# patngnw/NewsRecommendation

Hardware: AMD Instinct MI355X
Metric: train impressions/sec @ batch 512, NRMS (higher is better)
Workload: dtype bf16; 1 GPU; NRMS train step (fwd+bwd+Adam), MIND-small shapes: title_len=30, history=50, npratio=4, 300-d word table; per_gpu_batch=512, global_batch=512, vocab_rows=30000, freeze_embedding=False, compact_history=False, dense_batch=False, feed=resident, deterministic=False, optimizer=flat bucket + HIP fused Adam, parallelism=dp1

## Files before the change

### newsrecommendation_amd/csrc/nr_gemm.hip

```cpp
#include <stdlib.h>

#include "nr_gemm.h"

namespace {

constexpr int BM = 128, BN = 128, BK = 32, NTHR = 256;
constexpr int SC = BN + 4;

template <typename T> struct TileCfg {
  static constexpr int CH = 16 / (int)sizeof(T);
  static constexpr int SK = BK + CH;
  static constexpr int CPR = BK / CH;
  static constexpr int NCH = BM * CPR / NTHR;
  static constexpr int RPC = BM / CH;
  static constexpr size_t STAGE_BYTES = (size_t)2 * 2 * BM * SK * sizeof(T);
};
constexpr size_t EPI_BYTES = (size_t)64 * SC * sizeof(float);

template <typename T> constexpr size_t smem_bytes() {
  return TileCfg<T>::STAGE_BYTES > EPI_BYTES ? TileCfg<T>::STAGE_BYTES : EPI_BYTES;
}

union Chunk {
  uint4 u;
// ... 1919 lines not shown
          const int row = u / xc, ch = u - row * xc;
          *reinterpret_cast<uint4*>(a.dx + (r0 + row) * a.lddx + ch * 8) = make_uint4(0, 0, 0, 0);
        }
      if (near)
        for (int u = lane; u < L * qc; u += 64) {
          const int row = u / qc, ch = u - row * qc;
          *reinterpret_cast<uint4*>(a.dpre + (r0 + row) * a.ldp + ch * 8) = make_uint4(0, 0, 0, 0);
        }
    }
    nsteps = run;
  } else {
    for (int c = tid; c < nsteps; c += 512) sList[c] = b0 + c * G;
  }
  for (int c = tid; c < 256; c += 512) {
    sW2[c] = c < q ? a.w2[c] : 0.f;
    sRedW[c] = 0.f;
  }
  const int wcol0 = wid * TPW * 16;
  bf16x8 bfr[TPW][KS2];
#pragma unroll
  for (int t = 0; t < TPW; ++t) {
    const bf16_t* brow = a.w1t + (size_t)min(wcol0 + t * 16 + fr, N - 1) * a.ldw1t + 8 * g;
#pragma unroll
    for (int s2 = 0; s2 < KS2; ++s2) bfr[t][s2] = *reinterpret_cast<const bf16x8*>(brow + 32 * s2);
  }
  __builtin_amdgcn_s_waitcnt(0x0F70);
  __syncthreads();
  float* prow_out = a.partial + (size_t)blockIdx.x * (q + 1);
  if (nsteps == 0) {
    for (int c = tid; c <= q; c += 512) prow_out[c] = 0.f;
    return;
  }

  const uint32_t dump_lds = lds0 + Cfg::DUMP + wid * 1024;
  uint4* dump_g = g_nt_dump + wid * 64 + lane;
  auto issue_stage = [&](int kk) {
    const uint32_t slot = lds0 + (kk % NS) * STAGE;
    const bool real = kk < nsteps;
    const int sq = real ? sList[kk] : 0;
    const int row0 = sq * L;
#pragma unroll
    for (int u = 0; u < PW; ++u) {
      const int p = wid + NW * u;
      if (real && p < EPIECES) {
        const int i = p / KS2, s2 = p - i * KS2;
        const bf16_t* rp = a.e + (size_t)min(row0 + 16 * i + prow, M - 1) * a.lde + c8;
        dma16(rp + min(32 * s2, q - 8 - c8), slot + p * 1024);
      } else if (real && p < EPIECES + Cfg::GPIECES) {
        const int j = p - EPIECES;
        dma16(a.g + (size_t)sq * a.ldg + min(256 * j + 4 * lane, N - 4), slot + p * 1024);
      } else {
        dma16(a.e + c8, dump_lds);
      }
    }
  };
  const int ks0 = wid, ks1 = wid + NW;
  auto load_seq = [&](int kk, bf16x8 (&xf)[RT][2], float& al) {
    const int row0 = sList[kk < nsteps ? kk : 0] * L;
#pragma unroll
    for (int i = 0; i < RT; ++i) {
      const bf16_t* rp = a.x + (size_t)min(row0 + 16 * i + fr, M - 1) * a.ldx;
      xf[i][0] = *reinterpret_cast<const bf16x8*>(rp + min(32 * ks0 + 8 * g, N - 8));
      xf[i][1] = *reinterpret_cast<const bf16x8*>(rp + min(32 * ks1 + 8 * g, N - 8));
    }
    const int rowa = sList[(kk >= 1 && kk - 1 < nsteps) ? kk - 1 : 0] * L;
    al = a.alpha[min(rowa + (lane & 31), M - 1)];
  };
  auto g_frag = [&](const float* grow, int ks, bf16x8& hi, bf16x8& lo) {
    const int k0 = 32 * ks + 8 * g;
    const bool ok = ks < KS && k0 < N;
    const f32x4 v0 = *reinterpret_cast<const f32x4*>(grow + min(k0, N - 8));
    const f32x4 v1 = *reinterpret_cast<const f32x4*>(grow + min(k0, N - 8) + 4);
#pragma unroll
    for (int e2 = 0; e2 < 8; ++e2) {
      const float v = ok ? (e2 < 4 ? v0[e2] : v1[e2 - 4]) : 0.f;
      const bf16_t h = (bf16_t)v;
      hi[e2] = h;
      lo[e2] = (bf16_t)(v - (float)h);
    }
  };
  auto sum32 = [&](float v) {
    v += __builtin_bit_cast(float, __builtin_amdgcn_update_dpp(0, __builtin_bit_cast(int, v), 0x128, 0xf, 0xf, false));
    v += __builtin_bit_cast(float, __builtin_amdgcn_update_dpp(0, __builtin_bit_cast(int, v), 0x124, 0xf, 0xf, false));
    v += __builtin_bit_cast(float, __builtin_amdgcn_update_dpp(0, __builtin_bit_cast(int, v), 0x122, 0xf, 0xf, false));
    v += __builtin_bit_cast(float, __builtin_amdgcn_update_dpp(0, __builtin_bit_cast(int, v), 0x121, 0xf, 0xf, false));
    return v + __shfl_xor(v, 16, 64);
  };
  const int offA = fr * 64 + ((g ^ swzP(fr)) << 4);
  const uint32_t inv_qc = (uint32_t)((0x100000000ull + (uint32_t)qc - 1) / (uint32_t)qc);
  int brow[2], bcc[2];
#pragma unroll
  for (int j = 0; j < 2; ++j) {
    const uint32_t u = (uint32_t)(tid + 512 * j);
    uint32_t r = __umulhi(u, inv_qc);
    if (r * (uint32_t)qc > u) --r;
    brow[j] = (int)r;
    bcc[j] = (int)(u - r * (uint32_t)qc);
  }

  bf16x8 xf[RT][2];
  float al_nb, al_cur = 0.f;
  float* myacc = reinterpret_cast<float*>(smem + Cfg::ACCW) + tid * 8;
#pragma unroll
  for (int j = 0; j < 2; ++j) {
    *reinterpret_cast<f32x4*>(myacc + j * 4096) = (f32x4){0.f, 0.f, 0.f, 0.f};
    *reinterpret_cast<f32x4*>(myacc + j * 4096 + 4) = (f32x4){0.f, 0.f, 0.f, 0.f};
  }
  float accb = 0.f;

#pragma unroll 1
  for (int kk = 0; kk < 2; ++kk) issue_stage(kk);
  load_seq(0, xf, al_nb);

#pragma unroll 1
  for (int k = 0; k < nsteps + 2; ++k) {
    if (k >= 2) asm volatile("s_waitcnt vmcnt(%0)" ::"n"(Cfg::STEADY) : "memory");
    else wait_vmcnt_le(k == 0 ? PW + Cfg::LOADS : Cfg::OPS + Cfg::LOADS);
    __builtin_amdgcn_s_barrier();
    issue_stage(k + 2);
    auto phase_a = [&]()     {
      const bool real = k < nsteps;
      const float* grow = reinterpret_cast<const float*>(smem + (k % NS) * STAGE + EPIECES * 1024);
      f32x4 da[RT];
#pragma unroll
      for (int i = 0; i < RT; ++i) da[i] = (f32x4){0.f, 0.f, 0.f, 0.f};
      if (real) {
#pragma unroll
        for (int j = 0; j < 2; ++j) {
          bf16x8 hi, lo;
          g_frag(grow, j == 0 ? ks0 : ks1, hi, lo);
#pragma unroll
          for (int i = 0; i < RT; ++i) {
            da[i] = __builtin_amdgcn_mfma_f32_16x16x32_bf16(hi, xf[i][j], da[i], 0, 0, 0);
            da[i] = __builtin_amdgcn_mfma_f32_16x16x32_bf16(lo, xf[i][j], da[i], 0, 0, 0);
          }
        }
      }
      if (g == 0) {
#pragma unroll
        for (int i = 0; i < RT; ++i) sPartA[((k & 1) * NW + wid) * 32 + 16 * i + fr] = da[i][0];
      }
      al_cur = al_nb;
      load_seq(k + 1, xf, al_nb);
    };
    auto phase_b = [&]()     {
      const int kp = k - 1;
      const bool real = kp >= 0 && kp < nsteps;
      const int row0 = real ? sList[kp] * L : 0;
      const bool in = (lane & 31) < L;
      const float alv = in ? al_cur : 0.f;
      const float* part = sPartA + ((kp & 1) * NW) * 32 + (lane & 31);
      float dA = 0.f;
#pragma unroll
      for (int w = 0; w < NW; ++w) dA += part[w * 32];
      dA = in ? dA : 0.f;
      const float tsum = sum32(alv * dA);
      const float ds = alv * (dA - tsum);
      if (wid == 0 && lane < 32) sAlpha[(kp & 3) * 32 + lane] = alv;
      if (real) accb += sum32(ds);
      char* st = smem + ((kp + NS) % NS) * STAGE;
#pragma unroll
      for (int j = 0; j < 2; ++j) {
        const int row = brow[j], cc = bcc[j];
        const bool valid = real && row < L;
        const int rc = min(row, L - 1);
        const float dsr = __shfl(ds, rc, 64);
        const int eoff = ((rc >> 4) * KS2 + (cc >> 2)) * 1024 + (rc & 15) * 64 + (((cc & 3) ^ swzP(rc & 15)) << 4);
        const bf16x8 ev = *reinterpret_cast<const bf16x8*>(st + eoff);
        const f32x4 wa = *reinterpret_cast<const f32x4*>(sW2 + cc * 8), wb = *reinterpret_cast<const f32x4*>(sW2 + cc * 8 + 4);
        bf16x8 o;
        f32x4 a0 = *reinterpret_cast<const f32x4*>(myacc + j * 4096), a1 = *reinterpret_cast<const f32x4*>(myacc + j * 4096 + 4);
#pragma unroll
        for (int e2 = 0; e2 < 8; ++e2) {
          const float f = (float)ev[e2], wv = e2 < 4 ? wa[e2] : wb[e2 - 4];
          o[e2] = (bf16_t)(dsr * wv * (1.f - f * f));
          const float p = valid ? dsr * f : 0.f;
          if (e2 < 4) a0[e2] += p;
          else a1[e2 - 4] += p;
        }
        *reinterpret_cast<f32x4*>(myacc + j * 4096) = a0;
        *reinterpret_cast<f32x4*>(myacc + j * 4096 + 4) = a1;
        if (valid) *reinterpret_cast<bf16x8*>(st + eoff) = o;
        uint4* dst = valid ? reinterpret_cast<uint4*>(a.dpre + (size_t)(row0 + row) * a.ldp + cc * 8) : dump_g;
        *dst = __builtin_bit_cast(uint4, o);
      }
    };
    auto phase_c = [&]()     {
      const int kc = k - 2;
      const bool real = kc >= 0 && kc < nsteps;
      const int row0 = real ? sList[kc] * L : 0;
      const char* st = smem + ((kc + NS) % NS) * STAGE;
      const float* grow = reinterpret_cast<const float*>(st + EPIECES * 1024);
#pragma unroll
      for (int i = 0; i < RT; ++i) {
        f32x4 acc[TPW];
#pragma unroll
        for (int t = 0; t < TPW; ++t) acc[t] = (f32x4){0.f, 0.f, 0.f, 0.f};
        if (real && wcol0 < N) {
#pragma unroll
          for (int s2 = 0; s2 < KS2; ++s2) {
            const bf16x8 af = *reinterpret_cast<const bf16x8*>(st + (i * KS2 + s2) * 1024 + offA);
#pragma unroll
            for (int t = 0; t < TPW; ++t) acc[t] = __builtin_amdgcn_mfma_f32_16x16x32_bf16(bfr[t][s2], af, acc[t], 0, 0, 0);
          }
        }
        const int ml = 16 * i + fr;
        const bool rok = real && ml < L;
        const float al = sAlpha[((kc + 4) & 3) * 32 + ml];
        bf16_t* crow = a.dx + (size_t)(row0 + ml) * a.lddx;
#pragma unroll
        for (int t = 0; t < TPW; t += 2) {
          uint2 pk[2];
#pragma unroll
          for (int h = 0; h < 2; ++h) {
            const int lc = wcol0 + (t + h) * 16 + 4 * g;
            const f32x4 gq = *reinterpret_cast<const f32x4*>(grow + lc);
            const f32x4 v = acc[t + h];
            const bf16x4 o = {(bf16_t)(v[0] + al * gq[0]), (bf16_t)(v[1] + al * gq[1]), (bf16_t)(v[2] + al * gq[2]), (bf16_t)(v[3] + al * gq[3])};
            pk[h] = __builtin_bit_cast(uint2, o);
          }
          const auto s0 = __builtin_amdgcn_permlane16_swap(pk[0].x, pk[1].x, false, false);
          const auto s1 = __builtin_amdgcn_permlane16_swap(pk[0].y, pk[1].y, false, false);
          const int col = wcol0 + (t + (g & 1)) * 16 + (g >> 1) * 8;
          uint4* dst = (rok && col + 8 <= N) ? reinterpret_cast<uint4*>(crow + col) : dump_g;
          *dst = make_uint4(s0[0], s1[0], s0[1], s1[1]);
        }
      }
    };
    if (wid < NW / 2) {
      phase_a();
      phase_b();
      phase_c();
    } else {
      phase_c();
      phase_a();
      phase_b();
    }
  }
#pragma unroll
  for (int j = 0; j < 2; ++j)
#pragma unroll
    for (int e2 = 0; e2 < 8; ++e2) atomicAdd(sRedW + bcc[j] * 8 + e2, myacc[j * 4096 + e2]);
  __syncthreads();
  for (int c = tid; c < q; c += 512) prow_out[c] = sRedW[c];
  if (tid == 0) prow_out[q] = accb;
}

template <int EPI, int NT16, bool PK, int WM>
int launch_nt_dma_w(const RowSrc& A, const void* B, int ldb, int M, int N, int K, const EpiArgs& ep, hipStream_t stream) {
  constexpr int DBM = 64 * WM, NP = DBM / 16 + NT16, STAGE = NP * 1024, NS = dma_ring_stages(STAGE, WM);
  constexpr size_t ring = (size_t)NS * STAGE, epi = (size_t)32 * (NT16 * 16 + 4) * sizeof(float);
  constexpr size_t epk = PK ? (size_t)128 * (NT16 * 16 + 8) * sizeof(bf16_t) : 0;
  constexpr size_t gtile = EPI == EPI_POOLBWD && PK ? (size_t)((12 * NT16 * 16 * 4 + 1023) / 1024) * 1024 + 1024
                                                    : ((EPI == EPI_SCATTER || EPI == EPI_STORE) ? 2048 : 1024);
  constexpr size_t smem0 = ring > epi ? ring : epi, smem1 = smem0 > epk ? smem0 : epk, smem = smem1 + gtile;
  auto kern = gemm_nt_dma_kernel<EPI, NT16, PK, WM>;
  NR_CHECK_HIP(hipFuncSetAttribute(reinterpret_cast<const void*>(kern), hipFuncAttributeMaxDynamicSharedMemorySize, (int)smem));
  const int tilesM = (M + DBM - 1) / DBM, nchunks = (N + NT16 * 16 - 1) / (NT16 * 16);
  const int grid = ((tilesM + 7) / 8) * 8 * nchunks;
  hipLaunchKernelGGL(kern, dim3(grid), dim3(128 * WM), smem, stream, (const bf16_t*)A.base, A.ld, (const bf16_t*)B, ldb, M, N, K, ep, nchunks);
  NR_CHECK_LAUNCH();
  return NR_OK;
}

template <int EPI, int NT16, bool PK>
int launch_nt_dma_p(const RowSrc& A, const void* B, int ldb, int M, int N, int K, const EpiArgs& ep, hipStream_t stream) {
  constexpr bool fits2 = 3 * (8 + NT16) * 1024 <= 78 * 1024;
  if (fits2 && (N <= 2 * NT16 * 16 || K <= 224)) return launch_nt_dma_w<EPI, NT16, PK, 2>(A, B, ldb, M, N, K, ep, stream);
  return launch_nt_dma_w<EPI, NT16, PK, 4>(A, B, ldb, M, N, K, ep, stream);
}

template <int EPI, int NT16>
int launch_nt_dma_t(const RowSrc& A, const void* B, int ldb, int M, int N, int K, const EpiArgs& ep, hipStream_t stream) {
  if (EPI != EPI_SCATTER && ep.out_dtype == NR_BF16) return launch_nt_dma_p<EPI, NT16, true>(A, B, ldb, M, N, K, ep, stream);
  return launch_nt_dma_p<EPI, NT16, false>(A, B, ldb, M, N, K, ep, stream);
}

template <int NT16>
int launch_nt_dma_e(const RowSrc& A, const void* B, int ldb, int M, int N, int K, int epi, const EpiArgs& ep, hipStream_t s) {
  switch (epi) {
    case EPI_STORE: return launch_nt_dma_t<EPI_STORE, NT16>(A, B, ldb, M, N, K, ep, s);
    case EPI_STORE_TANH: return launch_nt_dma_t<EPI_STORE_TANH, NT16>(A, B, ldb, M, N, K, ep, s);
    case EPI_POOLBWD: return launch_nt_dma_t<EPI_POOLBWD, NT16>(A, B, ldb, M, N, K, ep, s);
    case EPI_SCATTER: return launch_nt_dma_t<EPI_SCATTER, NT16>(A, B, ldb, M, N, K, ep, s);
  }
  nr_set_error("gemm_nt_dma: bad epilogue %d", epi);
  return NR_ERR_ARG;
}

namespace tn3 {
using tn2::swz_a;
using tn2::tr_frag;
constexpr int TBM = 32, NS = 4;
template <int WK, int NI> struct Geo {
  static constexpr int TBN = 32 * NI, TBK = 80 * WK, NT = 128 * WK, NW = 2 * WK, CHA = TBN / 8, CH = TBK / 8, SCW = TBK + 4;
  static constexpr int PA = TBM * CHA / 64, PBP = TBM * CH / 64, NP = PA + PBP, STAGE = NP * 1024;
  static constexpr size_t RING = (size_t)NS * STAGE, EPI = (size_t)64 * SCW * sizeof(float);
  static constexpr size_t SMEM = RING > EPI ? RING : EPI;
};
template <int WK> __device__ __forceinline__ int swz_b(int row, int chunk) {
  return WK == 2 ? chunk ^ (2 * ((row >> 3) & 1)) : chunk ^ (4 * ((row >> 1) & 1) + 2 * ((row >> 3) & 1));
}

template <int WK, int NI>
__global__ __launch_bounds__(128 * WK) void gemm_tn3_kernel(const bf16_t* __restrict__ dC, int ldc, const bf16_t* __restrict__ X,
                                                            int ldx, float* __restrict__ dW, int ldw, float* __restrict__ db,
                                                            int M, int N, int K, int Nstore, int Kstore, int tilesK, int ntile,
                                                            int nsplit, int rps, const int32_t* __restrict__ slab_list,
                                                            const int32_t* __restrict__ slab_count, int xgap, float* __restrict__ scratch) {
  using G = Geo<WK, NI>;
  constexpr int TBN = G::TBN, TBK = G::TBK, NT = G::NT, NW = G::NW, CHA = G::CHA, CH = G::CH, SCW = G::SCW, PA = G::PA, NP = G::NP,
                STAGE = G::STAGE;
  constexpr int PB = NP / NW, PX = NP % NW;
  extern __shared__ __attribute__((aligned(16))) char smem[];
  const bool det = nr_fix_on();
  float* sC = reinterpret_cast<float*>(smem);
  const uint32_t lds0 = (uint32_t)(size_t)(__attribute__((address_space(3))) char*)smem;

  const int b = blockIdx.x, xcd = b & 7, local = b >> 3;
  const int split = (local / ntile) * 8 + xcd, tile = local % ntile;
  if (split >= nsplit) return;
  const int tn = tile / tilesK, tk = tile % tilesK;
  const int n0 = tn * TBN, k0 = tk * TBK;
  __shared__ int sSlab[1024];
  const bool slabs = slab_list != nullptr, counted = !slabs && slab_count != nullptr;
  int mbeg = split * rps, nk, kbeg = 0;
  if (slabs || counted) {
    const int total = counted ? (*slab_count + TBM - 1) / TBM : *slab_count, per = (total + nsplit - 1) / nsplit;
    kbeg = split * per;
    nk = min(per, total - kbeg);
    if (nk <= 0) return;
    if (slabs) {
      for (int i = threadIdx.x; i < nk; i += blockDim.x) sSlab[i] = slab_list[kbeg + i];
      __syncthreads();
    }
    mbeg = 0;
  } else {
    const int mend = min(M, mbeg + rps);
    if (mbeg >= mend) return;
    nk = (mend - mbeg) / TBM;
  }
  const int tid = threadIdx.x, lane = tid & 63;
  const int wid = __builtin_amdgcn_readfirstlane(tid >> 6), wm = wid / WK, wn = wid % WK;
  const bool extra = wid < PX;
  const int pfirst = wid * PB + min(wid, PX);
  const bool db_wave = (db != nullptr) && (tk == 0) && (wn == wm);

  const bf16_t* src[PB + 1];
  size_t adv[PB + 1];
  int xrow[PB + 1];
#pragma unroll
  for (int t = 0; t < PB + 1; ++t) {
    const int p = pfirst + t;
    xrow[t] = -1;
    if (p < PA) {
      const int P = 64 * p + lane, row = P / CHA, cpos = P - row * CHA;
      const int col = min(n0 + swz_a(row, cpos) * 8, N - 8);
      src[t] = dC + (size_t)(mbeg + row) * ldc + col;
      adv[t] = (size_t)TBM * ldc;
    } else {
      const int P = 64 * (p - PA) + lane, row = min(P / CH, TBM - 1), cpos = P - (P / CH) * CH;
      const int col = min(k0 + swz_b<WK>(row, cpos) * 8, K - 8);
      src[t] = X + (size_t)(mbeg + row) * ldx + col;
      adv[t] = (size_t)TBM * ldx;
      xrow[t] = mbeg + row;
    }
  }
  const uint32_t ginv = xgap > 0 ? (uint32_t)((0x100000000ull + (uint32_t)xgap - 1) / (uint32_t)xgap) : 0u;
  auto issue = [&](int stage, int kt) {
    const size_t sl = slabs ? (size_t)sSlab[kt] : (size_t)(kbeg + kt);
#pragma unroll
    for (int t = 0; t < PB + 1; ++t)
      if (t < PB || extra) {
        size_t off = sl * adv[t];
        if (xgap > 0 && xrow[t] >= 0) {
          const uint32_t m = (uint32_t)sl * TBM + (uint32_t)xrow[t];
          uint32_t q = __umulhi(m, ginv);
          if (q * (uint32_t)xgap > m) --q;
          off += (size_t)q * ldx;
        }
        dma16(src[t] + off, lds0 + stage * STAGE + (pfirst + t) * 1024);
      }
  };
  auto wait_stages = [&](int stages) {
    if (extra) {
      if (stages >= 2) asm volatile("s_waitcnt vmcnt(%0)" ::"n"(2 * (PB + 1)) : "memory");
      else if (stages == 1) asm volatile("s_waitcnt vmcnt(%0)" ::"n"(PB + 1) : "memory");
      else asm volatile("s_waitcnt vmcnt(0)" ::: "memory");
    } else {
      if (stages >= 2) asm volatile("s_waitcnt vmcnt(%0)" ::"n"(2 * PB) : "memory");
      else if (stages == 1) asm volatile("s_waitcnt vmcnt(%0)" ::"n"(PB) : "memory");
      else asm volatile("s_waitcnt vmcnt(0)" ::: "memory");
    }
  };

  f32x4 acc[NI][5];
#pragma unroll
  for (int i = 0; i < NI; ++i)
#pragma unroll
    for (int j = 0; j < 5; ++j) acc[i][j] = (f32x4){0.f, 0.f, 0.f, 0.f};
  f32x4 accdb = (f32x4){0.f, 0.f, 0.f, 0.f};
  const bf16_t one = (bf16_t)1.f, zero = (bf16_t)0.f;

  const int g = lane >> 4, q = (lane & 15) >> 2, pp = lane & 3;
  const int r0 = 8 * g + q, r1 = r0 + 4, off = 4 * (pp & 1);
  const int a0 = r0 * TBN + off, a1 = r1 * TBN + off, ca = wm * 2 * NI + (pp >> 1);
  int ob0[5], ob1[5];
#pragma unroll
  for (int j = 0; j < 5; ++j) {
    const int chunk = (wn * 80 + j * 16) / 8 + (pp >> 1);
    ob0[j] = TBM * TBN + r0 * TBK + swz_b<WK>(r0, chunk) * 8 + off;
    ob1[j] = TBM * TBN + r1 * TBK + swz_b<WK>(r1, chunk) * 8 + off;
  }

#pragma unroll
  for (int s = 0; s < NS - 1; ++s)
    if (s < nk) issue(s, s);
  for (int kt = 0; kt < nk; ++kt) {
    wait_stages(min(NS - 2, nk - 1 - kt));
    __builtin_amdgcn_s_barrier();
    if (kt + NS - 1 < nk) issue((kt + NS - 1) % NS, kt + NS - 1);
    const bf16_t* st = reinterpret_cast<const bf16_t*>(smem + (kt % NS) * STAGE);
    bf16x8 bf[5];
#pragma unroll
    for (int j = 0; j < 5; ++j) bf[j] = tr_frag(st + ob0[j], st + ob1[j]);
#pragma unroll
    for (int i = 0; i < NI; ++i) {
      const bf16x8 af = tr_frag(st + a0 + swz_a(r0, ca + 2 * i) * 8, st + a1 + swz_a(r1, ca + 2 * i) * 8);
#pragma unroll
      for (int j = 0; j < 5; ++j) acc[i][j] = __builtin_amdgcn_mfma_f32_16x16x32_bf16(af, bf[j], acc[i][j], 0, 0, 0);
      if (db_wave) {
        const bf16_t v = (lane & 15) == i ? one : zero;
        const bf16x8 sel = {v, v, v, v, v, v, v, v};
        accdb = __builtin_amdgcn_mfma_f32_16x16x32_bf16(sel, af, accdb, 0, 0, 0);
      }
    }
  }
  asm volatile("s_waitcnt vmcnt(0)" ::: "memory");
  __builtin_amdgcn_s_barrier();

  if (db_wave) {
#pragma unroll
    for (int e = 0; e < 4; ++e) {
      const int ti = 4 * (lane >> 4) + e, n = n0 + wm * 16 * NI + ti * 16 + (lane & 15);
      if (ti < NI && n < Nstore) nr_accum(db + n, accdb[e], det);
    }
  }
#pragma unroll
  for (int pass = 0; pass < TBN / 64; ++pass) {
    if (pass) __syncthreads();
    if (wm == pass / (NI / 4)) {
      const int ib = (pass % (NI / 4)) * 4;
#pragma unroll
      for (int j = 0; j < 5; ++j) {
        const int col = wn * 80 + j * 16 + (lane & 15);
#pragma unroll
        for (int i = 0; i < 4; ++i)
#pragma unroll
          for (int r = 0; r < 4; ++r) sC[(i * 16 + (lane >> 4) * 4 + r) * SCW + col] = acc[ib + i][j][r];
      }
    }
    __syncthreads();
    if (scratch != nullptr) {
      float* base = scratch + ((size_t)(split * ntile + tile) * TBN + pass * 64) * TBK;
      for (int u = tid; u < 64 * (TBK / 4); u += NT) {
        const int row = u / (TBK / 4), c4 = (u - row * (TBK / 4)) * 4;
        *reinterpret_cast<f32x4*>(base + (size_t)row * TBK + c4) = *reinterpret_cast<const f32x4*>(sC + row * SCW + c4);
      }
      continue;
    }
    for (int u = tid; u < 64 * TBK; u += NT) {
      const int row = u / TBK, c = u - row * TBK;
      const int n = n0 + pass * 64 + row, k = k0 + c;
      if (n < Nstore && k < Kstore) nr_accum(dW + (size_t)n * ldw + k, sC[row * SCW + c], det);
    }
  }
}

__global__ __launch_bounds__(256) void tn3_reduce_kernel(const float* __restrict__ scratch, float* __restrict__ dW, int ldw, int Nstore, int Kstore,
                                                         int TBN, int TBK, int tilesK, int ntile, int nsplit, int mode,
                                                         const int32_t* __restrict__ count) {
  __shared__ f32x4 sAcc[4][64];
  int active = nsplit;
  if (mode != 0) {
    const int total = mode == 2 ? (*count + TBM - 1) / TBM : *count, per = (total + nsplit - 1) / nsplit;
    active = per > 0 ? (total + per - 1) / per : 0;
  }
  const int k4n = (Kstore + 3) / 4, o = threadIdx.x & 63, sg = threadIdx.x >> 6;
  const size_t sstride = (size_t)ntile * TBN * TBK;
  for (int u0 = blockIdx.x * 64; u0 < Nstore * k4n; u0 += gridDim.x * 64) {
    const int u = u0 + o;
    const bool ok = u < Nstore * k4n;
    const int n = ok ? u / k4n : 0, k = ok ? (u - n * k4n) * 4 : 0;
    const int tile = (n / TBN) * tilesK + k / TBK;
    const float* p = scratch + ((size_t)tile * TBN + n % TBN) * TBK + k % TBK;
    f32x4 a0 = (f32x4){0.f, 0.f, 0.f, 0.f}, a1 = a0;
    int sp = sg;
    for (; sp + 4 < active; sp += 8) {
      const f32x4 v0 = *reinterpret_cast<const f32x4*>(p + (size_t)sp * sstride);
      const f32x4 v1 = *reinterpret_cast<const f32x4*>(p + (size_t)(sp + 4) * sstride);
      a0[0] += v0[0]; a0[1] += v0[1]; a0[2] += v0[2]; a0[3] += v0[3];
      a1[0] += v1[0]; a1[1] += v1[1]; a1[2] += v1[2]; a1[3] += v1[3];
    }
    if (sp < active) {
      const f32x4 v0 = *reinterpret_cast<const f32x4*>(p + (size_t)sp * sstride);
      a0[0] += v0[0]; a0[1] += v0[1]; a0[2] += v0[2]; a0[3] += v0[3];
    }
    sAcc[sg][o] = (f32x4){a0[0] + a1[0], a0[1] + a1[1], a0[2] + a1[2], a0[3] + a1[3]};
    __syncthreads();
    if (sg == 0 && ok) {
      const f32x4 b0 = sAcc[0][o], b1 = sAcc[1][o], b2 = sAcc[2][o], b3 = sAcc[3][o];
      float* d = dW + (size_t)n * ldw + k;
#pragma unroll
      for (int e = 0; e < 4; ++e)
        if (k + e < Kstore) d[e] += (b0[e] + b1[e]) + (b2[e] + b3[e]);
    }
    __syncthreads();
  }
}

template <int WK, int NI>
size_t scratch_floats_t(int M, int N, int K) {
  using G = Geo<WK, NI>;
  const int tilesN = (N + G::TBN - 1) / G::TBN, tilesK = (K + G::TBK - 1) / G::TBK, ntile = tilesN * tilesK;
  const int resident = 256 * (WK == 4 ? 1 : 2);
  int nsplit = (resident / ntile / 8) * 8;
  if (nsplit < 8) nsplit = 8;
  return (size_t)(nsplit + 8) * ntile * G::TBN * G::TBK;
}

template <int WK, int NI>
int launch_t(const void* dC, int ldc, const void* X, int ldx, float* dW, int ldw, float* db, int M, int N, int K, int Nstore,
             int Kstore, hipStream_t stream, const int32_t* slab_list = nullptr, const int32_t* slab_count = nullptr, int xgap = 0,
             float* scratch = nullptr, size_t scratch_floats = 0) {
  using G = Geo<WK, NI>;
  const int tilesN = (N + G::TBN - 1) / G::TBN, tilesK = (K + G::TBK - 1) / G::TBK, ntile = tilesN * tilesK;
  const int resident = 256 * (WK == 4 ? 1 : 2);
  int nsplit = (resident / ntile / 8) * 8;
  if (nsplit < 8) nsplit = 8;
  int rps = (M + nsplit - 1) / nsplit;
  rps = ((rps + TBM - 1) / TBM) * TBM;
  if (rps < 16 * TBM) rps = 16 * TBM;
  nsplit = (M + rps - 1) / rps;
  const int grid = ((nsplit + 7) / 8) * 8 * ntile;
  auto kern = gemm_tn3_kernel<WK, NI>;
  NR_CHECK_HIP(hipFuncSetAttribute(reinterpret_cast<const void*>(kern), hipFuncAttributeMaxDynamicSharedMemorySize, (int)G::SMEM));
  const bool counted = slab_list == nullptr && slab_count != nullptr;
  if (slab_list != nullptr && (M / TBM + nsplit - 1) / nsplit > 1024) slab_list = nullptr;
  const bool use_scratch = scratch != nullptr && scratch_floats >= (size_t)nsplit * ntile * G::TBN * G::TBK && (((uintptr_t)scratch) & 15) == 0;
  hipLaunchKernelGGL(kern, dim3(grid), dim3(G::NT), G::SMEM, stream, (const bf16_t*)dC, ldc, (const bf16_t*)X, ldx, dW, ldw, db, M, N,
                     K, Nstore, Kstore, tilesK, ntile, nsplit, rps, slab_list, (slab_list || counted) ? slab_count : nullptr, xgap,
                     use_scratch ? scratch : nullptr);
  if (use_scratch) {
    const int mode = slab_list != nullptr ? 1 : (counted ? 2 : 0);
    int rg = (Nstore * ((Kstore + 3) / 4) + 63) / 64;
    if (rg > 4096) rg = 4096;
    hipLaunchKernelGGL(tn3_reduce_kernel, dim3(rg), dim3(256), 0, stream, (const float*)scratch, dW, ldw, Nstore, Kstore, G::TBN, G::TBK, tilesK,
                       ntile, nsplit, mode, mode ? slab_count : nullptr);
  }
  NR_CHECK_LAUNCH();
  return NR_OK;
}

constexpr int MIN_M = 16384;
bool eligible(int ldc, int ldx, int M, int N, int K) {
  return M % TBM == 0 && M >= MIN_M && N >= 8 && K >= 8 && N % 8 == 0 && K % 8 == 0 && ldc % 8 == 0 && ldx % 8 == 0;
}
bool wide_k(int K) { return K > 160 && ((K + 319) / 320) * 320 * 100 <= K * 115; }
int launch(const void* dC, int ldc, const void* X, int ldx, float* dW, int ldw, float* db, int M, int N, int K, int Nstore,
           int Kstore, hipStream_t stream, const int32_t* slab_list = nullptr, const int32_t* slab_count = nullptr, int xgap = 0,
           float* scratch = nullptr, size_t sf = 0) {
  if (wide_k(K)) {
    if (N > 256) return launch_t<4, 8>(dC, ldc, X, ldx, dW, ldw, db, M, N, K, Nstore, Kstore, stream, slab_list, slab_count, xgap, scratch, sf);
    return launch_t<4, 4>(dC, ldc, X, ldx, dW, ldw, db, M, N, K, Nstore, Kstore, stream, slab_list, slab_count, xgap, scratch, sf);
  }
  return launch_t<2, 4>(dC, ldc, X, ldx, dW, ldw, db, M, N, K, Nstore, Kstore, stream, slab_list, slab_count, xgap, scratch, sf);
}
size_t scratch_floats(int M, int N, int K) {
  if (N < 8 || K < 8) return 0;
  if (wide_k(K)) return N > 256 ? scratch_floats_t<4, 8>(M, N, K) : scratch_floats_t<4, 4>(M, N, K);
  return scratch_floats_t<2, 4>(M, N, K);
}
}

template <typename T, int KIND, int EPI>
int launch_nt_t(const RowSrc& A, const void* B, int ldb, int M, int N, int K, const EpiArgs& ep, hipStream_t stream) {
  const int tilesM = (M + BM - 1) / BM, tilesN = (N + BN - 1) / BN;
  const int grid = ((tilesM + 7) / 8) * 8 * tilesN;
  auto kern = gemm_nt_kernel<T, KIND, EPI>;
  const size_t smem = smem_bytes<T>();
  int rc = set_smem(kern, smem);
  if (rc) return rc;
  hipLaunchKernelGGL(kern, dim3(grid), dim3(NTHR), smem, stream, A, (const T*)B, ldb, M, N, K, ep, tilesM, tilesN);
  NR_CHECK_LAUNCH();
  return NR_OK;
}

template <typename T, int KIND>
int launch_nt_k(const RowSrc& A, const void* B, int ldb, int M, int N, int K, int epi, const EpiArgs& ep, hipStream_t s) {
  switch (epi) {
    case EPI_STORE: return launch_nt_t<T, KIND, EPI_STORE>(A, B, ldb, M, N, K, ep, s);
    case EPI_STORE_TANH: return launch_nt_t<T, KIND, EPI_STORE_TANH>(A, B, ldb, M, N, K, ep, s);
    case EPI_POOLBWD: return launch_nt_t<T, KIND, EPI_POOLBWD>(A, B, ldb, M, N, K, ep, s);
    case EPI_SCATTER: return launch_nt_t<T, KIND, EPI_SCATTER>(A, B, ldb, M, N, K, ep, s);
  }
  nr_set_error("gemm_nt: bad epilogue %d", epi);
  return NR_ERR_ARG;
}

template <typename T>
int launch_nt_d(const RowSrc& A, const void* B, int ldb, int M, int N, int K, int epi, const EpiArgs& ep, hipStream_t s) {
  switch (A.kind) {
    case ROWS_DENSE: return launch_nt_k<T, ROWS_DENSE>(A, B, ldb, M, N, K, epi, ep, s);
    case ROWS_GATHER: return launch_nt_k<T, ROWS_GATHER>(A, B, ldb, M, N, K, epi, ep, s);
    case ROWS_IM2COL3:
      if (epi == EPI_STORE) return launch_nt_t<T, ROWS_IM2COL3, EPI_STORE>(A, B, ldb, M, N, K, ep, s);
      if (epi == EPI_STORE_TANH) return launch_nt_t<T, ROWS_IM2COL3, EPI_STORE_TANH>(A, B, ldb, M, N, K, ep, s);
      break;
  }
  nr_set_error("gemm_nt: unsupported row source %d / epilogue %d", A.kind, epi);
  return NR_ERR_ARG;
}

template <typename T, int KIND>
int launch_tn_t(const void* dC, int ldc, const RowSrc& A, float* dW, int ldw, float* db, int M, int N, int K, int Nstore,
                int Kstore, hipStream_t stream) {
  const int tilesN = (N + BM - 1) / BM, tilesK = (K + BN - 1) / BN;
  int splits = (256 * 4 + tilesN * tilesK - 1) / (tilesN * tilesK);
  int rps = (M + splits - 1) / splits;
  rps = ((rps + BK - 1) / BK) * BK;
  if (rps < 8 * BK) rps = 8 * BK;
  splits = (M + rps - 1) / rps;
  auto kern = gemm_tn_kernel<T, KIND>;
  const size_t smem = smem_bytes<T>();
  int rc = set_smem(kern, smem);
  if (rc) return rc;
  hipLaunchKernelGGL(kern, dim3(tilesN * tilesK, splits), dim3(NTHR), smem, stream, (const T*)dC, ldc, A, dW, ldw, db, M, N,
                     K, Nstore, Kstore, tilesK, rps);
  NR_CHECK_LAUNCH();
  return NR_OK;
}

template <typename T>
int launch_tn_d(const void* dC, int ldc, const RowSrc& A, float* dW, int ldw, float* db, int M, int N, int K, int Nstore,
                int Kstore, hipStream_t s) {
  switch (A.kind) {
    case ROWS_DENSE: return launch_tn_t<T, ROWS_DENSE>(dC, ldc, A, dW, ldw, db, M, N, K, Nstore, Kstore, s);
    case ROWS_GATHER: return launch_tn_t<T, ROWS_GATHER>(dC, ldc, A, dW, ldw, db, M, N, K, Nstore, Kstore, s);
    case ROWS_IM2COL3: return launch_tn_t<T, ROWS_IM2COL3>(dC, ldc, A, dW, ldw, db, M, N, K, Nstore, Kstore, s);
  }
  nr_set_error("gemm_tn: bad row source %d", A.kind);
  return NR_ERR_ARG;
}

}

template <typename T>
__global__ __launch_bounds__(256) void im2col3_materialize_kernel(RowSrc A, T* __restrict__ out, int ldo, int M) {
  constexpr int CH = 16 / (int)sizeof(T);
  const int Dp = A.ld, cpr = Dp / CH, T_ = A.Tlen;
  const size_t total = (size_t)M * cpr;
  const uint4 zero = make_uint4(0, 0, 0, 0);
  for (size_t u = (size_t)blockIdx.x * blockDim.x + threadIdx.x; u < total; u += (size_t)gridDim.x * blockDim.x) {
    const int m = (int)(u / cpr), d = (int)(u - (size_t)m * cpr) * CH;
    const int blk = m / T_, t = m - blk * T_;
    const uint4 v = load_rows_chunk<T, ROWS_IM2COL3>(A, m, Dp + d, M, 3 * Dp);
    T* o = out + (size_t)m * ldo + d;
    *reinterpret_cast<uint4*>(o + Dp) = v;
    if (t + 1 < T_) *reinterpret_cast<uint4*>(o + ldo) = v;
    else *reinterpret_cast<uint4*>(o + 2 * Dp) = zero;
    if (t > 0) *reinterpret_cast<uint4*>(o - ldo + 2 * Dp) = v;
    else *reinterpret_cast<uint4*>(o) = zero;
  }
}

template <typename T>
__global__ __launch_bounds__(256) void im2col3_title_kernel(RowSrc A, T* __restrict__ out, int ldo, int M, const int32_t* __restrict__ needed,
                                                            int n, int margin) {
  constexpr int CH = 16 / (int)sizeof(T);
  const int Dp = A.ld, cpr = Dp / CH, T_ = A.Tlen, blk = blockIdx.x;
  __shared__ int near;
  if (threadIdx.x == 0) near = 0;
  __syncthreads();
  for (int t = max(0, blk - margin) + (int)threadIdx.x; t <= min(n - 1, blk + margin); t += 256)
    if (needed[t] != 0) near = 1;
  __syncthreads();
  if (!near) return;
  const uint4 zero = make_uint4(0, 0, 0, 0);
  for (int u = threadIdx.x; u < T_ * cpr; u += 256) {
    const int t = u / cpr, d = (u - t * cpr) * CH, m = blk * T_ + t;
    if (m >= M) break;
    const uint4 v = load_rows_chunk<T, ROWS_IM2COL3>(A, m, Dp + d, M, 3 * Dp);
    T* o = out + (size_t)m * ldo + d;
    *reinterpret_cast<uint4*>(o + Dp) = v;
    if (t + 1 < T_) *reinterpret_cast<uint4*>(o + ldo) = v;
    else *reinterpret_cast<uint4*>(o + 2 * Dp) = zero;
    if (t > 0) *reinterpret_cast<uint4*>(o - ldo + 2 * Dp) = v;
    else *reinterpret_cast<uint4*>(o) = zero;
  }
}

template <typename T>
__global__ __launch_bounds__(256) void conv_rows_kernel(RowSrc A, T* __restrict__ out, int n, const int32_t* __restrict__ needed, int margin) {
  constexpr int CH = 16 / (int)sizeof(T);
  const int Dp = A.ld, cpr = Dp / CH, T_ = A.Tlen, blk = blockIdx.x;
  if (needed != nullptr) {
    __shared__ int near;
    if (threadIdx.x == 0) near = 0;
    __syncthreads();
    for (int t = max(0, blk - margin) + (int)threadIdx.x; t <= min(n - 1, blk + margin); t += 256)
      if (needed[t] != 0) near = 1;
    __syncthreads();
    if (!near) return;
  }
  const uint4 zero = make_uint4(0, 0, 0, 0);
  T* o0 = out + (size_t)blk * (T_ + 1) * Dp;
  for (int u = threadIdx.x; u < (T_ + 2) * cpr; u += 256) {
    const int r = u / cpr, d = (u - r * cpr) * CH;
    uint4 v = zero;
    if (r >= 1 && r <= T_) v = load_rows_chunk<T, ROWS_IM2COL3>(A, blk * T_ + r - 1, Dp + d, n * T_, 3 * Dp);
    *reinterpret_cast<uint4*>(o0 + (size_t)r * Dp + d) = v;
  }
}

template <typename T>
__global__ __launch_bounds__(256) void gather_title_kernel(RowSrc A, T* __restrict__ out, int ldo, int M, int K, int L,
                                                           const int32_t* __restrict__ needed, int n, int margin,
                                                           const int32_t* __restrict__ keep_all) {
  constexpr int CH = 16 / (int)sizeof(T);
  const int cpr = K / CH, blk = blockIdx.x;
  __shared__ int near;
  if (threadIdx.x == 0) near = *keep_all != 0 ? 1 : 0;
  __syncthreads();
  for (int t = max(0, blk - margin) + (int)threadIdx.x; t <= min(n - 1, blk + margin); t += 256)
    if (needed[t] != 0) near = 1;
  for (int t = threadIdx.x; t < L; t += 256)
    if (blk * L + t < M && A.ids[(size_t)(blk * L + t) * A.ids_stride] != 0) near = 1;
  __syncthreads();
  if (!near) return;
// ... 873 lines not shown
```

Before: 176,700 impressions/s.

## Software-pipeline LDS fragment loads and use scalar-base DMA in tn3 weight-grad GEMM

Restructures the gemm_tn3 main loop so LDS fragments for the next k-tile are double-buffered in registers and loaded while the current tile's MFMAs run. In 8-wave configs half the waves issue loads before their MFMAs and half after, staggering LDS traffic. Global-to-LDS DMA now uses a wave-uniform scalar base plus 32-bit per-lane offsets, which removes per-lane 64-bit pointer arrays and most of the per-row gap division. The cost is higher register pressure and 32-bit offsets that could overflow for large strides.

```diff
diff --git a/newsrecommendation_amd/csrc/nr_gemm.hip b/newsrecommendation_amd/csrc/nr_gemm.hip
--- a/newsrecommendation_amd/csrc/nr_gemm.hip
+++ b/newsrecommendation_amd/csrc/nr_gemm.hip
@@ -2245,6 +2245,19 @@
   return WK == 2 ? chunk ^ (2 * ((row >> 3) & 1)) : chunk ^ (4 * ((row >> 1) & 1) + 2 * ((row >> 3) & 1));
 }
 
+__device__ __forceinline__ void dma16s(const void* base, uint32_t voff, uint32_t lds_dst) {
+  uint32_t keep;
+  asm volatile("s_mov_b32 %0, m0\n\ts_mov_b32 m0, %3\n\ts_nop 0\n\tglobal_load_lds_dwordx4 %1, %2\n\ts_mov_b32 m0, %0"
+               : "=&s"(keep)
+               : "v"(voff), "s"(base), "s"(__builtin_amdgcn_readfirstlane(lds_dst))
+               : "memory");
+}
+__device__ __forceinline__ uint32_t udiv_inv(uint32_t m, uint32_t inv, uint32_t d) {
+  uint32_t q = __umulhi(m, inv);
+  if (q * d > m) --q;
+  return q;
+}
+
 template <int WK, int NI>
 __global__ __launch_bounds__(128 * WK) void gemm_tn3_kernel(const bf16_t* __restrict__ dC, int ldc, const bf16_t* __restrict__ X,
                                                             int ldx, float* __restrict__ dW, int ldw, float* __restrict__ db,
@@ -2289,40 +2302,43 @@
   const int pfirst = wid * PB + min(wid, PX);
   const bool db_wave = (db != nullptr) && (tk == 0) && (wn == wm);
 
-  const bf16_t* src[PB + 1];
-  size_t adv[PB + 1];
-  int xrow[PB + 1];
+  uint32_t loff[PB + 1];
 #pragma unroll
   for (int t = 0; t < PB + 1; ++t) {
     const int p = pfirst + t;
-    xrow[t] = -1;
     if (p < PA) {
       const int P = 64 * p + lane, row = P / CHA, cpos = P - row * CHA;
       const int col = min(n0 + swz_a(row, cpos) * 8, N - 8);
-      src[t] = dC + (size_t)(mbeg + row) * ldc + col;
-      adv[t] = (size_t)TBM * ldc;
+      loff[t] = (uint32_t)(row * ldc + col) * 2u;
     } else {
       const int P = 64 * (p - PA) + lane, row = min(P / CH, TBM - 1), cpos = P - (P / CH) * CH;
       const int col = min(k0 + swz_b<WK>(row, cpos) * 8, K - 8);
-      src[t] = X + (size_t)(mbeg + row) * ldx + col;
-      adv[t] = (size_t)TBM * ldx;
-      xrow[t] = mbeg + row;
+      loff[t] = (uint32_t)(row * ldx + col) * 2u;
     }
   }
   const uint32_t ginv = xgap > 0 ? (uint32_t)((0x100000000ull + (uint32_t)xgap - 1) / (uint32_t)xgap) : 0u;
   auto issue = [&](int stage, int kt) {
-    const size_t sl = slabs ? (size_t)sSlab[kt] : (size_t)(kbeg + kt);
+    const int sl = slabs ? __builtin_amdgcn_readfirstlane(sSlab[kt]) : kbeg + kt;
+    const size_t m0 = (size_t)mbeg + (size_t)sl * TBM;
+    const bf16_t *gc = dC + m0 * ldc, *gx = X + m0 * ldx;
+    uint32_t q0 = 0;
+    if (xgap > 0) {
+      q0 = udiv_inv((uint32_t)m0, ginv, (uint32_t)xgap);
+      gx += (size_t)q0 * ldx;
+    }
 #pragma unroll
     for (int t = 0; t < PB + 1; ++t)
       if (t < PB || extra) {
-        size_t off = sl * adv[t];
-        if (xgap > 0 && xrow[t] >= 0) {
-          const uint32_t m = (uint32_t)sl * TBM + (uint32_t)xrow[t];
-          uint32_t q = __umulhi(m, ginv);
-          if (q * (uint32_t)xgap > m) --q;
-          off += (size_t)q * ldx;
+        const int p = pfirst + t;
+        const bool isx = p >= PA;
+        uint32_t o = loff[t];
+        if (xgap > 0 && isx) {
+          int ln = lane;
+          asm volatile("" : "+v"(ln));
+          const uint32_t m = (uint32_t)m0 + (uint32_t)min((64 * (p - PA) + ln) / CH, TBM - 1);
+          o += (udiv_inv(m, ginv, (uint32_t)xgap) - q0) * (uint32_t)ldx * 2u;
         }
-        dma16(src[t] + off, lds0 + stage * STAGE + (pfirst + t) * 1024);
+        dma16s(isx ? gx : gc, o, lds0 + stage * STAGE + p * 1024);
       }
   };
   auto wait_stages = [&](int stages) {
@@ -2359,25 +2375,75 @@
 #pragma unroll
   for (int s = 0; s < NS - 1; ++s)
     if (s < nk) issue(s, s);
-  for (int kt = 0; kt < nk; ++kt) {
-    wait_stages(min(NS - 2, nk - 1 - kt));
-    __builtin_amdgcn_s_barrier();
-    if (kt + NS - 1 < nk) issue((kt + NS - 1) % NS, kt + NS - 1);
+  constexpr bool STAG = NW == 8;
+  constexpr int PFB = (STAG && NI == 8) ? 0 : 5, NHI = 5 - PFB;
+  const bool ahead = !STAG || wid >= NW / 2;
+  bf16x8 fb_lo[2][PFB ? PFB : 1], fb_hi[NHI ? NHI : 1], fa0[2];
+  int xa0 = a0 + swz_a(r0, ca) * 8, xa1 = a1 + swz_a(r1, ca) * 8;
+  auto read_a = [&](const bf16_t* st, int i) { return tr_frag(st + (xa0 ^ (16 * i)), st + (xa1 ^ (16 * i))); };
+  auto load_lo = [&](int buf, int kt) {
     const bf16_t* st = reinterpret_cast<const bf16_t*>(smem + (kt % NS) * STAGE);
-    bf16x8 bf[5];
-#pragma unroll
-    for (int j = 0; j < 5; ++j) bf[j] = tr_frag(st + ob0[j], st + ob1[j]);
+    fa0[buf] = read_a(st, 0);
+#pragma unroll
+    for (int j = 0; j < PFB; ++j) fb_lo[buf][j] = tr_frag(st + ob0[j], st + ob1[j]);
+  };
+  auto load_hi = [&](int kt) {
+    const bf16_t* st = reinterpret_cast<const bf16_t*>(smem + (kt % NS) * STAGE);
+#pragma unroll
+    for (int j = PFB; j < 5; ++j) fb_hi[j - PFB] = tr_frag(st + ob0[j], st + ob1[j]);
+  };
+  auto mfmas = [&](int buf, int kt) {
+    const bf16_t* st = reinterpret_cast<const bf16_t*>(smem + (kt % NS) * STAGE);
+    bf16x8 af = fa0[buf];
+    asm volatile("" : "+v"(xa0), "+v"(xa1));
 #pragma unroll
     for (int i = 0; i < NI; ++i) {
-      const bf16x8 af = tr_frag(st + a0 + swz_a(r0, ca + 2 * i) * 8, st + a1 + swz_a(r1, ca + 2 * i) * 8);
-#pragma unroll
-      for (int j = 0; j < 5; ++j) acc[i][j] = __builtin_amdgcn_mfma_f32_16x16x32_bf16(af, bf[j], acc[i][j], 0, 0, 0);
+      bf16x8 nx = af;
+      if (i + 1 < NI) nx = read_a(st, i + 1);
+#pragma unroll
+      for (int j = 0; j < 5; ++j)
+        acc[i][j] = __builtin_amdgcn_mfma_f32_16x16x32_bf16(af, j < PFB ? fb_lo[buf][j < PFB ? j : 0] : fb_hi[j < PFB ? 0 : j - PFB], acc[i][j], 0, 0, 0);
       if (db_wave) {
         const bf16_t v = (lane & 15) == i ? one : zero;
         const bf16x8 sel = {v, v, v, v, v, v, v, v};
         accdb = __builtin_amdgcn_mfma_f32_16x16x32_bf16(sel, af, accdb, 0, 0, 0);
       }
-    }
+      af = nx;
+    }
+  };
+  auto step = [&](int kt, int cur) {
+    __builtin_amdgcn_s_waitcnt(0xC07F);
+    const bool more = kt + 1 < nk;
+    if (more) {
+      wait_stages(min(NS - 3, nk - 2 - kt));
+      __builtin_amdgcn_s_barrier();
+    }
+    if (ahead && more) {
+      if (kt + NS - 1 < nk) issue((kt + NS - 1) % NS, kt + NS - 1);
+      load_lo(cur ^ 1, kt + 1);
+    }
+    __builtin_amdgcn_sched_barrier(0);
+    mfmas(cur, kt);
+    __builtin_amdgcn_sched_barrier(0);
+    if (more) {
+      if (!ahead) {
+        if (kt + NS - 1 < nk) issue((kt + NS - 1) % NS, kt + NS - 1);
+        load_lo(cur ^ 1, kt + 1);
+      }
+      if (NHI) load_hi(kt + 1);
+    }
+  };
+  wait_stages(min(NS - 2, nk - 1));
+  __builtin_amdgcn_s_barrier();
+  load_lo(0, 0);
+  if (NHI) load_hi(0);
+  {
+    int kt = 0;
+    for (; kt + 1 < nk; kt += 2) {
+      step(kt, 0);
+      step(kt + 1, 1);
+    }
+    if (kt < nk) step(kt, 0);
   }
   asm volatile("s_waitcnt vmcnt(0)" ::: "memory");
   __builtin_amdgcn_s_barrier();
```

Result: no change. 176,600 impressions/s (-0.1%).
